# 10XGenomics/thermite

Hardware: AMD Instinct MI355X
Metric: aligned reads/sec (91 bp) (higher is better)
Workload: dtype i32

## Files before the change

thermite_amd/capi.py:

```python
import ctypes as C
import os

import numpy as np

from .refdata import EXON_DT, REF_DT, SPAN_DT, TX_DT

_HERE = os.path.dirname(os.path.abspath(__file__))
SO_PATH = os.environ.get("THM_LIB") or os.path.join(_HERE, "_build", "libthermite_amd.so")

MEM_DT = np.dtype([("ref_idx", "<u8"), ("query_idx", "<u4"), ("len", "<u4")])
ALN_DT = np.dtype(
    [
        ("ystart", "<u8"),
        ("yend", "<u8"),
        ("ylen", "<u8"),
        ("ops_off", "<u8"),
        ("tx_ystart", "<u8"),
        ("tx_yend", "<u8"),
        ("tx_ylen", "<u8"),
        ("tx_ops_off", "<u8"),
        ("score", "<i4"),
        ("ref_id", "<u4"),
        ("xstart", "<u4"),
        ("xend", "<u4"),
# ... 1075 lines not shown
        status = (_copy(v.hit_status, v.n_hits, "<i4") if v.hit_status else np.zeros(int(v.n_hits), "<i4"))
        return _copy(v.alns, v.n_hits, ALN_DT), _copy(v.ops, v.n_op_bytes, np.uint8), status

    def counters(self):
        out = np.zeros(N_COUNTERS, "<u8")
        self._chk(lib().thm_counters_get(self.h, _ptr(out)))
        return out

    def reset_counters(self):
        self._chk(lib().thm_counters_reset(self.h))

    def counters_allreduce(self, comm):
        self._chk(lib().thm_counters_allreduce(self.h, comm.h))

    def counters_device_ptr(self):
        return lib().thm_counters_device_ptr(self.h)

    def timings(self):
        out = np.zeros(N_TIMINGS, "<f4")
        self._chk(lib().thm_timings_get(self.h, _ptr(out)))
        return dict(zip(TIMING_NAMES, out.tolist()))

    def debug_prof(self, reset=True):
        out = np.zeros(16, "<u8")
        self._chk(lib().thm_debug_prof_get(self.h, _ptr(out), int(reset)))
        return out

    def debug_set_pool_caps(self, smem_cap=0, cand_cap=0, ops_cap=0):
        n = C.c_uint32()
        self._chk(lib().thm_debug_set_pool_caps(self.h, smem_cap, cand_cap, ops_cap, C.byref(n)))
        return n.value

    def debug_set_flags(self, tpr=None, rounds=0, seed_infer=None, seed_stats=None, seed_direct=None, finish_exact=None,
                        finish_subst=None):
        word = (0 if tpr is None else (2 if tpr else 1)) | (int(rounds) << 8)
        word |= 0 if seed_infer is None else (16 if seed_infer else 4)
        word |= 0 if seed_stats is None else (8 if seed_stats else 32)
        word |= 0 if seed_direct is None else (128 if seed_direct else 64)
        word |= 0 if finish_exact is None else (0x2000 if finish_exact else 0x1000)
        word |= 0 if finish_subst is None else (0x8000 if finish_subst else 0x4000)
        self._chk(lib().thm_debug_set_flags(self.h, word))

    def debug_seed_stats(self):
        out = np.zeros(2, "<u8")
        self._chk(lib().thm_debug_seed_stats(self.h, _ptr(out)))
        return int(out[0]), int(out[1])

    def debug_smem_finish_stats(self):
        out = np.zeros(4, "<u8")
        self._chk(lib().thm_debug_smem_finish_stats(self.h, _ptr(out)))
        return tuple(int(x) for x in out)

    def debug_seed_direct_stats(self):
        out = np.zeros(4, "<u8")
        self._chk(lib().thm_debug_seed_direct_stats(self.h, _ptr(out)))
        return tuple(int(x) for x in out)

    def debug_fetch_lut(self, like):
        out = np.zeros_like(like)
        self._chk(lib().thm_debug_fetch_lut(self.h, _ptr(out), out.nbytes))
        return out

    def debug_set_band_clip(self, max_bw=None):
        self._chk(lib().thm_debug_set_band_clip(self.h, 0 if max_bw is None else int(max_bw) + 1))

    def debug_tpr_stats(self):
        out = np.zeros(32, "<u8")
        self._chk(lib().thm_debug_tpr_stats(self.h, _ptr(out)))
        return out

    def debug_knobs(self):
        out = np.zeros(16, "<u4")
        self._chk(lib().thm_debug_knobs(self.h, _ptr(out)))
# ... 222 lines not shown
```

thermite_amd/csrc/aligner.hip:

```cpp
#include <hip/hip_runtime.h>

#include <algorithm>
#include <cstdarg>
#include <cstdio>
#include <cstdlib>
#include <cstring>
#include <mutex>
#include <string>
#include <type_traits>
#include <vector>

#include "aligner_internal.h"
#include "lut_direct.h"

namespace thm {
const char* global_error_cstr();
}
using namespace thm;

static int swg_blocks_per_cu() {
  static const int v = [] {
    const char* e = getenv("THM_SWG_BPC");
    const int v = e ? atoi(e) : 4;
    return (v >= 1 && v <= 8) ? v : 4;
// ... 476 lines not shown

int32_t thm_debug_prof_get(thm_aligner* a, uint64_t out[16], int32_t reset) {
  if (!a || !out) return THM_ERR_INVALID_ARG;
  HIPCHK(a, hipSetDevice(a->device));
  unsigned long long* p = a->d_counters + 2 * THM_N_COUNTERS;
  HIPCHK(a, hipMemcpyAsync(out, p, 16 * 8, hipMemcpyDeviceToHost, a->stream));
  if (reset) HIPCHK(a, hipMemsetAsync(p, 0, 16 * 8, a->stream));
  HIPCHK(a, hipStreamSynchronize(a->stream));
  return THM_OK;
}

int32_t thm_debug_set_pool_caps(thm_aligner* a, uint64_t smem_cap, uint64_t cand_cap, uint64_t ops_cap, uint32_t* n_replays) {
  if (!a) return THM_ERR_INVALID_ARG;
  a->dbg_smem_cap = smem_cap;
  a->dbg_cand_cap = cand_cap;
  a->dbg_ops_cap = ops_cap;
  a->seed.smem_cap = a->ext.cand_cap = a->ext.cand_ops_cap = 0;
  if (n_replays) *n_replays = a->n_replays;
  return THM_OK;
}

int32_t thm_debug_set_flags(thm_aligner* a, uint32_t flags) {
  if (!a) return THM_ERR_INVALID_ARG;
  if (flags & 1u) a->tpr.use_tpr = false;
  if (flags & 2u) a->tpr.use_tpr = true;
  const int r = (int)((flags >> 8) & 15u);
  if (r >= 1 && r <= TPR_MAX_ROUNDS) a->tpr.tpr_rounds = r;
  if (flags & 4u) a->dbg_seed_noinfer = true;
  if (flags & 16u) a->dbg_seed_noinfer = false;
  if (flags & 8u) a->dbg_seed_stats = true;
  if (flags & 32u) a->dbg_seed_stats = false;
  if (flags & 64u) a->dbg_seed_nodirect = true;
  if (flags & 128u) a->dbg_seed_nodirect = false;
  if (flags & 0x1000u) a->fin_classes &= ~1u;
  if (flags & 0x2000u) a->fin_classes |= 1u;
  if (flags & 0x4000u) a->fin_classes &= ~2u;
  if (flags & 0x8000u) a->fin_classes |= 2u;
  return THM_OK;
}
int32_t thm_debug_smem_finish_stats(thm_aligner* a, uint64_t stats[4]) {
  if (!a || !stats) return THM_ERR_INVALID_ARG;
  stats[0] = stats[1] = stats[2] = stats[3] = 0;
  if (!a->fin_blocks || !a->ext.finstats.get()) return THM_OK;
  HIPCHK(a, hipSetDevice(a->device));
  HIPCHK(a, hipStreamSynchronize(a->stream));
  std::vector<unsigned long long> rows((size_t)a->fin_blocks * 4);
  HIPCHK(a, hipMemcpy(rows.data(), a->ext.finstats, rows.size() * 8, hipMemcpyDeviceToHost));
  for (size_t b = 0; b < a->fin_blocks; b++)
    for (int k = 0; k < 4; k++) stats[k] += rows[b * 4 + k];
  return THM_OK;
}
int32_t thm_debug_seed_stats(thm_aligner* a, uint64_t stats[2]) {
  if (!a || !stats) return THM_ERR_INVALID_ARG;
  stats[0] = stats[1] = 0;
  if (!a->s_work_counts.p || a->s_work_counts.cap < 128) return THM_OK;
  HIPCHK(a, hipSetDevice(a->device));
  HIPCHK(a, hipStreamSynchronize(a->stream));
  HIPCHK(a, hipMemcpy(stats, a->s_work_counts + 8, 16, hipMemcpyDeviceToHost));
  return THM_OK;
}
int32_t thm_debug_seed_direct_stats(thm_aligner* a, uint64_t stats[4]) {
  if (!a || !stats) return THM_ERR_INVALID_ARG;
  stats[0] = stats[1] = stats[2] = stats[3] = 0;
  if (!a->dix) return THM_OK;
  stats[0] = a->dix->lut_direct ? 1 : 0;
  stats[1] = a->dix->lut_tagged;
// ... 75 lines not shown
```

thermite_amd/csrc/aligner_internal.h:

```cpp
#ifndef THERMITE_ALIGNER_INTERNAL_H
#define THERMITE_ALIGNER_INTERNAL_H
#include <hip/hip_runtime.h>

#include <cstdarg>
#include <cstdio>
#include <string>
#include <type_traits>
#include <vector>

#include "launch.h"
#include "thermite_internal.h"


struct DBuf {
  void* p = nullptr;
  size_t cap = 0;
  DBuf() = default;
  DBuf(const DBuf&) = delete;
  DBuf& operator=(const DBuf&) = delete;
  ~DBuf() { release(); }
  hipError_t ensure(size_t bytes) {
    if (bytes <= cap) return hipSuccess;
    release();
    size_t want = bytes + bytes / 4 + 256;
// ... 333 lines not shown
  Event ev_fork, ev_join;
  thm_align_opts opts;
  thm_align_opts run_opts;
  std::string err;

  DArr<unsigned long long> d_counters;
  DBuf d_ctl;
  static constexpr size_t CTL_WORK_COUNTS = 0, CTL_CURSORS = 128, CTL_FAULT = 192, CTL_QUEUE = 256,
                          CTL_QUEUE_EXT = CTL_QUEUE + thm::QUEUE_BYTES, CTL_BYTES = CTL_QUEUE_EXT + thm::QUEUE_BYTES;
  static_assert(CTL_BYTES % 16 == 0 && thm::QUEUE_BYTES % 16 == 0, "the block is zeroed 16 bytes at a time");
  DView<unsigned int> d_queue;
  DView<unsigned int> d_queue_ext;
  DView<int> d_fault;
  DView<unsigned long long> d_cursors;
  DView<unsigned long long> s_work_counts;
  DBuf b0, b1, b2, b3, b4, b5, b6, b7, b8;
  DArr<uint64_t> stage_scan_tmp;

  ReadsState reads;
  uint64_t n_reads = 0, n_bases = 0;
  uint32_t max_read_len = 0;
  std::vector<std::pair<uint32_t, uint64_t>> len_hist;
  uint64_t n_over = 0;
  bool uploaded = false;
  SeedState seed;
  ExtendState ext;
  uint64_t n_slow_host = 0;
  uint32_t fast_max_len = 0, slow_max_len = 0;
  OutputState out;
  uint64_t dbg_smem_cap = 0, dbg_cand_cap = 0, dbg_ops_cap = 0;
  uint32_t dbg_band_clip = 0;
  bool dbg_seed_noinfer = false, dbg_seed_stats = false;
  bool dbg_seed_nodirect = false;
  uint32_t fin_classes = 3;
  const void* ops_run_ptr = nullptr;
  size_t ops_run_cap = 0;
  uint32_t ops_run_half = 0;
  uint32_t fin_run_classes = 0, fin_blocks = 0;
  uint32_t n_replays = 0;
  bool ran = false, synced = false;
  Event ev[6];
  float timings[THM_N_TIMINGS] = {0};

  std::vector<uint64_t> h_off;
  std::vector<thm_aln> h_alns;
  std::vector<uint8_t> h_ops;
  std::vector<thm_mem> h_mems;
  std::vector<thm_swg_aln> h_swg;
  std::vector<thm_lr_aln> h_lr;
  SeedHitState sh;
  std::vector<thm_aln> h_hit_alns;
  std::vector<int32_t> h_hit_status;
  std::vector<uint8_t> h_hit_ops;
  CigarState cig;
  BamState bam;
  BgzfState bgzf;
  FastqState fq;
  InflateState fz;
  GzipState gz;
};

inline int fail(thm_aligner* a, int code, const char* fmt, ...) {
  char buf[512];
  va_list ap;
  va_start(ap, fmt);
  vsnprintf(buf, sizeof buf, fmt, ap);
// ... 99 lines not shown
```

thermite_amd/csrc/kernels_seed.hip:

```cpp
#include <hip/hip_runtime.h>

#include <algorithm>

#include "launch.h"
#include "lut_direct.h"
#include "swg_device.h"

namespace thm {
namespace dev {

__device__ __forceinline__ int base_code(uint8_t c) {
  return c == 'A' ? 0 : c == 'C' ? 1 : c == 'G' ? 2 : c == 'T' ? 3 : -1;
}
__device__ __forceinline__ uint8_t sanitize_base(uint8_t c) {
  if (c >= 'a' && c <= 'z') c = (uint8_t)(c - 32);
  return (c == 'A' || c == 'C' || c == 'G' || c == 'T' || c == 'N') ? c : (uint8_t)0;
}
__device__ __forceinline__ uint64_t load8_global(const uint8_t* p) {
  uint64_t v;
  __builtin_memcpy(&v, p, 8);
  return v;
}
__device__ __forceinline__ uint64_t load8_lds(const uint8_t* base16, int off) {
  const uint64_t* q = (const uint64_t*)(base16 + (off & ~7));
  const unsigned sh = (unsigned)(off & 7) * 8u;
  const uint64_t w0 = q[0], w1 = q[1];
  return sh ? ((w0 >> sh) | (w1 << (64u - sh))) : w0;
}

template <bool PROBE>
__device__ __forceinline__ int lcp_cmp(const uint8_t* tp, const uint8_t* q, int cap, bool* less) {
  *less = false;
  int o = 0;
  if (PROBE && cap > 0) {
    const uint64_t tw = load8_global(tp), qw = load8_global(q);
    const uint64_t x = tw ^ qw;
    if (x) {
      const int idx = __builtin_ctzll(x) >> 3;
// ... 161 lines not shown

__device__ __forceinline__ void sanitize16(const uint8_t* in, uint8_t* out, uint64_t n, uint64_t n_padded, uint64_t i) {
  if (i >= n_padded) return;
  uint4 v = make_uint4(0, 0, 0, 0);
  if (i < n) v = *(const uint4*)(in + i);
  uint32_t w[4] = {v.x, v.y, v.z, v.w};
#pragma unroll
  for (int j = 0; j < 4; j++) {
    uint32_t r = 0;
#pragma unroll
    for (int b = 0; b < 4; b++) {
      const uint64_t at = i + (uint64_t)(4 * j + b);
      const uint8_t c = (at < n) ? sanitize_base((uint8_t)(w[j] >> (8 * b))) : (uint8_t)0;
      r |= (uint32_t)c << (8 * b);
    }
    w[j] = r;
  }
  *(uint4*)(out + i) = make_uint4(w[0], w[1], w[2], w[3]);
}
__global__ void sanitize_kernel(const uint8_t* in, uint8_t* out, uint64_t n, uint64_t n_padded) {
  sanitize16(in, out, n, n_padded, ((uint64_t)blockIdx.x * blockDim.x + threadIdx.x) * 16);
}
__global__ void sanitize_reset_kernel(const uint8_t* in, uint8_t* out, uint64_t n, uint64_t n_padded, RunResetParams rp) {
  const uint64_t t = (uint64_t)blockIdx.x * blockDim.x + threadIdx.x;
  const uint4 zero = make_uint4(0, 0, 0, 0);
  if (t < rp.status_vec4) rp.status[t] = zero;
  if (t < rp.ctl_vec4) rp.ctl[t] = zero;
  if (t < THM_N_COUNTERS) rp.counters[THM_N_COUNTERS + t] = rp.counters[t];
  if (t == 0) *rp.san_head = zero;
  sanitize16(in, out, n, n_padded, t * 16);
}

constexpr int PROBE_STRIDE = 8;

__device__ __forceinline__ void block_append(bool flag, unsigned long long value, unsigned long long* list,
                                             unsigned long long* count) {
  __shared__ unsigned w_cnt[4];
  __shared__ unsigned long long b_base;
  const unsigned long long m = __ballot(flag);
  const int lane = lane_id(), wv = (int)(threadIdx.x >> 6);
  if (lane == 0) w_cnt[wv] = (unsigned)__popcll(m);
  __syncthreads();
  if (threadIdx.x == 0) {
    const unsigned total = w_cnt[0] + w_cnt[1] + w_cnt[2] + w_cnt[3];
    b_base = total ? atomicAdd(count, (unsigned long long)total) : 0ull;
  }
  __syncthreads();
  unsigned before = 0;
  for (int w = 0; w < wv; w++) before += w_cnt[w];
  if (flag) list[b_base + before + (unsigned long long)__popcll(m & ((1ull << lane) - 1ull))] = value;
  __syncthreads();
}

__device__ __forceinline__ unsigned* seed_stats_lds() {
  __shared__ unsigned s_cnt[4];
  return s_cnt;
}
__device__ __forceinline__ void seed_stats_begin() {
  unsigned* c = seed_stats_lds();
  if (threadIdx.x == 0) c[0] = c[1] = c[2] = c[3] = 0;
  __syncthreads();
}
__device__ __forceinline__ void seed_stats_note(int how) {
  const unsigned long long here = __ballot(1), dec = __ballot(how == MS_DECIDED);
  const unsigned long long dir = __ballot(how == MS_DIRECT), one = __ballot(how == MS_SA_ONE);
  if (lane_id() == (int)__builtin_ctzll(here)) {
    unsigned* c = seed_stats_lds();
    if (dec) atomicAdd(&c[0], (unsigned)__popcll(dec));
    if (here & ~dec) atomicAdd(&c[1], (unsigned)__popcll(here & ~dec));
    if (dir) atomicAdd(&c[2], (unsigned)__popcll(dir));
    if (one) atomicAdd(&c[3], (unsigned)__popcll(one));
  }
}
template <class C>
__device__ __forceinline__ void seed_stats_end(const SeedParamsT<C>& p) {
  unsigned* c = seed_stats_lds();
  __syncthreads();
  if (threadIdx.x == 0) {
    if (c[0]) atomicAdd(&p.work_counts[8], (unsigned long long)c[0]);
    if (c[1]) atomicAdd(&p.work_counts[9], (unsigned long long)c[1]);
    if (c[2]) atomicAdd(&p.work_counts[10], (unsigned long long)c[2]);
    if (c[3]) atomicAdd(&p.work_counts[11], (unsigned long long)c[3]);
  }
}

template <class C>
__device__ __forceinline__ int probe_store(const SeedParamsT<C>& p, const uint8_t* rd, int L, int pos, uint64_t item0, int hint,
                                           bool& decided) {
  const int k = (int)p.min_seed_len;
  int d = 0;
  C lo = 0, hi = 0;
  const int how = ms_search(p.ix, rd, L, pos, k, hint, !(p.flags & SEED_NODIRECT), d, lo, hi);
  decided = how == MS_DECIDED;
  if (p.flags & SEED_STATS) seed_stats_note(how);
  const int e = (d >= k) ? pos + d : 0;
  const uint64_t item = item0 + (uint64_t)pos;
  p.ms_end[item] = (uint16_t)e;
  if (hint == 0 || e > hint) {
    p.ms_lo[item] = lo;
    p.ms_hi[item] = hi;
  }
  return e;
}

template <class C>
__global__ __launch_bounds__(256) void seed_first_kernel(SeedParamsT<C> p) {
  const uint64_t read = (uint64_t)blockIdx.x * 256 + threadIdx.x;
  const int lane = lane_id();
  const bool active = read < p.reads.n_reads;
  const int k = (int)p.min_seed_len;
  if (p.flags & SEED_STATS) seed_stats_begin();
  int d = 0, L = 0, how = MS_FULL;
  C lo = 0, hi = 0;
  bool too_long = false;
  if (active) {
    const uint64_t r0 = p.reads.offsets[read];
    const uint64_t Lfull = p.reads.offsets[read + 1] - r0;
    too_long = Lfull > MAX_READ_LEN;
    L = too_long ? 0 : (int)Lfull;
    if (too_long) p.read_status[read] = THM_ERR_UNSUPPORTED;
    if (k <= L) how = ms_search(p.ix, p.reads.bases + r0, L, 0, k, 0, !(p.flags & SEED_NODIRECT), d, lo, hi);
    if (L > 0) {
      const uint64_t item = ms_row(r0, read);
      p.ms_end[item] = (uint16_t)((d >= k) ? d : 0);
      p.ms_lo[item] = lo;
      p.ms_hi[item] = hi;
    }
// ... 31 lines not shown
      }
      hits = (unsigned long long)(hi - lo);
      p.read_smem_off[read] = slot;
      p.read_smem_cnt[read] = 1u;
      p.read_hits[read] = hits;
    }
    for (int o = 32; o > 0; o >>= 1) hits += __shfl_xor(hits, o);
    if (lane == leader) {
      if (!fits) atomicExch(p.fault, 1);
      atomicAdd(&p.counters[THM_CNT_SMEMS], (unsigned long long)__popcll(m));
      atomicAdd(&p.counters[THM_CNT_HITS], hits);
    }
  }
}

template <class C>
__global__ __launch_bounds__(256) void seed_grid_kernel(SeedParamsT<C> p, const unsigned long long* list,
                                                        const unsigned long long* count, uint32_t G) {
  const uint64_t tid = (uint64_t)blockIdx.x * 256 + threadIdx.x;
  const uint64_t wi = tid / G;
  if (p.flags & SEED_STATS) seed_stats_begin();
  if (wi < *count) {
    const uint64_t read = list[wi];
    const int g = (int)(tid - wi * G);
    const uint64_t r0 = p.reads.offsets[read];
    const int L = (int)(p.reads.offsets[read + 1] - r0);
    const int k = (int)p.min_seed_len;
    const int npos = L - k + 1;
    const int pos = (g + 1 == (int)G) ? npos - 1 : g * PROBE_STRIDE;
    if (!(pos <= 0 || pos >= npos || (g + 1 != (int)G && pos == npos - 1))) {
      const uint64_t item0 = ms_row(r0, read);
      const int hint = (p.flags & SEED_INFER) ? (int)p.ms_end[item0] : 0;
      bool decided;
      (void)probe_store(p, p.reads.bases + r0, L, pos, item0, hint, decided);
    }
  }
  if (p.flags & SEED_STATS) seed_stats_end(p);
}

template <class C>
__global__ __launch_bounds__(256) void seed_grid_cells_kernel(SeedParamsT<C> p, const unsigned long long* list,
                                                              const unsigned long long* count, uint32_t G) {
  __shared__ uint16_t s_end[256];
  const unsigned per = 256u / G;
  const unsigned rl = threadIdx.x / G;
  const int g = (int)(threadIdx.x - rl * G);
  const uint64_t wi = (uint64_t)blockIdx.x * per + rl;
  const bool live = rl < per && wi < *count;
  if (p.flags & SEED_STATS) seed_stats_begin();
  uint64_t read = 0, item0 = 0;
  int npos = 0, e = 0;
  if (live) {
    read = list[wi];
    const uint64_t r0 = p.reads.offsets[read];
    const int L = (int)(p.reads.offsets[read + 1] - r0);
    npos = L - (int)p.min_seed_len + 1;
    item0 = ms_row(r0, read);
    const int pos = (g + 1 == (int)G) ? npos - 1 : g * PROBE_STRIDE;
    const int e0 = p.ms_end[item0];
    if (pos <= 0) {
      e = e0;
    } else if (pos < npos && !(g + 1 != (int)G && pos == npos - 1)) {
      bool decided;
      e = probe_store(p, p.reads.bases + r0, L, pos, item0, (p.flags & SEED_INFER) ? e0 : 0, decided);
    }
  }
  s_end[threadIdx.x] = (uint16_t)e;
  __syncthreads();
  bool todo = false;
  if (live && g + 1 < (int)G) {
    const int a = g * PROBE_STRIDE, b = min(a + PROBE_STRIDE, npos - 1);
    if (b - a > 1) {
      const int ea = e, eb = s_end[rl * G + (unsigned)(b == npos - 1 ? (int)G - 1 : g + 1)];
      if (ea != 0 && ea == eb) {
        for (int q = a + 1; q < b; q++) p.ms_end[item0 + (uint64_t)q] = (uint16_t)ea;
      } else {
        todo = true;
      }
    }
  }
  block_append(todo, (read << 16) | (unsigned long long)g, p.work_cells, &p.work_counts[1]);
  if (p.flags & SEED_STATS) seed_stats_end(p);
}

template <class C>
__global__ __launch_bounds__(256) void seed_cells_kernel(SeedParamsT<C> p, const unsigned long long* list,
                                                         const unsigned long long* count, uint32_t NC) {
  const uint64_t tid = (uint64_t)blockIdx.x * 256 + threadIdx.x;
  const uint64_t wi = tid / NC;
  bool todo = false;
  uint64_t read = 0;
  int c = 0;
  if (wi < *count) {
    read = list[wi];
    c = (int)(tid - wi * NC);
    const uint64_t r0 = p.reads.offsets[read];
    const int L = (int)(p.reads.offsets[read + 1] - r0);
    const int npos = L - (int)p.min_seed_len + 1;
    const int a = c * PROBE_STRIDE, b = min(a + PROBE_STRIDE, npos - 1);
    if (b - a > 1) {
      const uint64_t item0 = ms_row(r0, read);
      const int ea = p.ms_end[item0 + (uint64_t)a], eb = p.ms_end[item0 + (uint64_t)b];
      if (ea != 0 && ea == eb) {
        for (int q = a + 1; q < b; q++) p.ms_end[item0 + (uint64_t)q] = (uint16_t)ea;
      } else {
        todo = true;
      }
    }
  }
  block_append(todo, (read << 16) | (unsigned long long)c, p.work_cells, &p.work_counts[1]);
}

template <class C>
__device__ __forceinline__ bool fill_item(const SeedParamsT<C>& p, uint64_t tid, uint64_t& read, int& pos, uint64_t& r0, int& L) {
  const int j = (int)(tid % PROBE_STRIDE);
  if (j == 0) return false;
  const unsigned long long w = p.work_cells[tid / PROBE_STRIDE];
  read = w >> 16;
  const int c = (int)(w & 0xffffu);
  r0 = p.reads.offsets[read];
  L = (int)(p.reads.offsets[read + 1] - r0);
  const int npos = L - (int)p.min_seed_len + 1;
  pos = c * PROBE_STRIDE + j;
  return pos < min(c * PROBE_STRIDE + PROBE_STRIDE, npos - 1);
}
template <class C>
__device__ __forceinline__ int fill_hint(const SeedParamsT<C>& p, uint64_t item0, int pos) {
  const int steps = ((int)p.min_seed_len + PROBE_STRIDE - 1) / PROBE_STRIDE + 1;
  int a = pos & ~(PROBE_STRIDE - 1);
  for (int s0 = 0; s0 < steps && a >= 0; s0 += 4, a -= 4 * PROBE_STRIDE) {
    int e[4];
#pragma unroll
    for (int u = 0; u < 4; u++) {
      const int at = a - u * PROBE_STRIDE;
      e[u] = (at >= 0 && s0 + u < steps) ? (int)p.ms_end[item0 + (uint64_t)at] : 0;
    }
#pragma unroll
    for (int u = 0; u < 4; u++)
      if (e[u] != 0) return e[u];
  }
  return 0;
}
template <class C>
__device__ __forceinline__ void fill_probe(const SeedParamsT<C>& p, uint64_t read, int pos, uint64_t r0, int L) {
  const uint64_t item0 = ms_row(r0, read);
  const int hint = (p.flags & SEED_INFER) ? fill_hint(p, item0, pos) : 0;
  bool decided;
  (void)probe_store(p, p.reads.bases + r0, L, pos, item0, hint, decided);
}

template <class C>
__global__ __launch_bounds__(256) void seed_fill_kernel(SeedParamsT<C> p) {
  const uint64_t total = p.work_counts[1] * PROBE_STRIDE;
  const uint64_t step = (uint64_t)gridDim.x * 256;
  if (p.flags & SEED_STATS) seed_stats_begin();
  for (uint64_t tid = (uint64_t)blockIdx.x * 256 + threadIdx.x; tid < total; tid += step) {
    uint64_t read, r0;
    int pos, L;
    if (fill_item(p, tid, read, pos, r0, L)) fill_probe(p, read, pos, r0, L);
  }
  if (p.flags & SEED_STATS) seed_stats_end(p);
}

template <class C>
__global__ __launch_bounds__(256) void seed_fill_keys_kernel(SeedParamsT<C> p) {
  const uint64_t total = p.work_counts[1] * PROBE_STRIDE;
  const uint64_t step = (uint64_t)gridDim.x * 256;
  for (uint64_t tid = (uint64_t)blockIdx.x * 256 + threadIdx.x; tid < total; tid += step) {
    uint64_t read, r0;
    int pos, L;
    uint16_t key = 0xFFFF;
    if (fill_item(p, tid, read, pos, r0, L)) {
      const uint64_t w0 = load8_global(p.reads.bases + r0 + pos);
      uint32_t code = 0;
      bool acgt = true;
      for (int t = 0; t < FILL_KEY_BASES; t++) {
        const int c = base_code((uint8_t)((w0 >> (8 * t)) & 0xff));
        acgt = acgt && (c >= 0);
        code = (code << 2) | (uint32_t)(c & 3);
      }
      key = (uint16_t)(acgt ? code : FILL_BUCKETS);
      atomicAdd(&p.fill_hist[key], 1u);
    }
    p.fill_keys[tid] = key;
  }
}
__global__ __launch_bounds__(1024) void seed_fill_scan_kernel(unsigned int* hist) {
  __shared__ unsigned part[1024];
  constexpr unsigned NB = FILL_BUCKETS + 1, PER = (NB + 1023) / 1024;
  const unsigned t = threadIdx.x, b0 = t * PER;
  unsigned sum = 0;
  for (unsigned k = 0; k < PER; k++)
// ... 420 lines not shown
    const uint32_t P = (max_len >= k) ? max_len - k + 1 : 1;
    return (P + dev::PROBE_STRIDE - 1) / dev::PROBE_STRIDE;
  };
  hipError_t e;
  hipLaunchKernelGGL(dev::seed_first_kernel<C>, blocks(n), dim3(256), 0, s, p);
  if ((e = hipGetLastError()) != hipSuccess) return e;
  const uint64_t n_short = n - p.n_long;
  struct Cls {
    uint64_t n;
    uint32_t max_len;
    const unsigned long long* list;
    const unsigned long long* count;
    bool fused;
  } cls[2] = {{n_short, p.max_len_short, p.work_short, p.work_counts + 0, true},
              {p.n_long, p.max_len_long, p.work_long, p.work_counts + 4, false}};
  uint64_t fill_cells = 0;
  for (const Cls& c : cls) {
    if (c.n == 0 || c.max_len < k + 1) continue;
    const uint64_t NC = cells_of(c.max_len), G = NC + 1;
    if (c.fused && G <= 256) {
      const uint64_t per = 256 / G;
      hipLaunchKernelGGL(dev::seed_grid_cells_kernel<C>, dim3((unsigned)((c.n + per - 1) / per)), dim3(256), 0, s, p, c.list, c.count,
                         (uint32_t)G);
      if ((e = hipGetLastError()) != hipSuccess) return e;
    } else {
      hipLaunchKernelGGL(dev::seed_grid_kernel<C>, blocks(c.n * G), dim3(256), 0, s, p, c.list, c.count, (uint32_t)G);
      if ((e = hipGetLastError()) != hipSuccess) return e;
      hipLaunchKernelGGL(dev::seed_cells_kernel<C>, blocks(c.n * NC), dim3(256), 0, s, p, c.list, c.count, (uint32_t)NC);
      if ((e = hipGetLastError()) != hipSuccess) return e;
    }
    fill_cells += c.n * NC;
  }
  if (fill_cells) {
    const dim3 worst = blocks(fill_cells * dev::PROBE_STRIDE);
    const dim3 fixed(std::min<unsigned>(worst.x, 256u * 8u * 4u));
    if (p.fill_mode == 2 && fill_cells * dev::PROBE_STRIDE < (1ull << 32)) {
      hipLaunchKernelGGL(dev::seed_fill_keys_kernel<C>, fixed, dim3(256), 0, s, p);
      hipLaunchKernelGGL(dev::seed_fill_scan_kernel, dim3(1), dim3(1024), 0, s, p.fill_hist);
      hipLaunchKernelGGL(dev::seed_fill_scatter_kernel<C>, fixed, dim3(256), 0, s, p);
      hipLaunchKernelGGL(dev::seed_fill_bucketed_kernel<C>, fixed, dim3(256), 0, s, p);
    } else {
      hipLaunchKernelGGL(dev::seed_fill_kernel<C>, p.fill_mode == 1 ? fixed : worst, dim3(256), 0, s, p);
    }
    if ((e = hipGetLastError()) != hipSuccess) return e;
  }
  auto select_waves = [&](const unsigned long long* list, const unsigned long long* count, unsigned int* queue, uint32_t max_len,
                          int nb) -> hipError_t {
    const uint32_t lcap = sel_lcap(max_len);
    const size_t lds = 4 * (size_t)lcap * (2 * sizeof(C) + 8);
    if (lds <= SEED_SELECT_LDS_LIMIT) {
      hipLaunchKernelGGL((dev::seed_select_kernel<C, false>), dim3(nb), dim3(256), lds, s, p, list, count, queue, lcap);
    } else {
      hipLaunchKernelGGL((dev::seed_select_kernel<C, true>), dim3(nb), dim3(256), 0, s, p, list, count, queue, lcap);
    }
    return hipGetLastError();
  };
  if (n_short) {
    unsigned long long* over_list = p.work_cells;
    unsigned long long* over_count = p.work_counts + 3;
    hipLaunchKernelGGL(dev::seed_select_thread_kernel<C>, dim3((unsigned)((n_short + 255) / 256)), dim3(256),
                       (size_t)256 * (2 * sizeof(C) + 4) * dev::SEL_CAP, s, p, over_list, over_count);
    if ((e = hipGetLastError()) != hipSuccess) return e;
    if ((e = select_waves(over_list, over_count, p.queue, p.max_len_short, std::min(n_blocks, 256))) != hipSuccess) return e;
  }
  if (p.n_long) {
    const int nb = (int)std::min<uint64_t>((uint64_t)n_blocks, (p.n_long + 3) / 4);
    if ((e = select_waves(p.work_long, p.work_counts + 4, p.queue + 1, p.max_len_long, std::max(nb, 1))) != hipSuccess) return e;
  }
  return hipSuccess;
}
hipError_t launch_seed(const SeedParamsT<uint32_t>& p, int n_blocks, hipStream_t s) { return launch_seed_t(p, n_blocks, s); }
hipError_t launch_seed(const SeedParamsT<uint64_t>& p, int n_blocks, hipStream_t s) { return launch_seed_t(p, n_blocks, s); }

template <class C>
static hipError_t launch_plan_pack_t(const PlanParams& pl, const PackParamsT<C>& pk, hipStream_t s) {
// ... 19 lines not shown
```

thermite_amd/csrc/launch.h:

```cpp
#ifndef THERMITE_LAUNCH_H
#define THERMITE_LAUNCH_H

#include <hip/hip_runtime.h>

#include "../../include/thermite_io.h"
#include "extend_plan.h"
#include "thermite_internal.h"

namespace thm {

template <class K, class P>
hipError_t launch_with_lds(K kern, unsigned n_blocks, unsigned threads, size_t lds, hipStream_t s, const P& p) {
  if (lds > 48 * 1024) {
    hipError_t e = hipFuncSetAttribute((const void*)kern, hipFuncAttributeMaxDynamicSharedMemorySize, (int)lds);
    if (e != hipSuccess) return e;
  }
  hipLaunchKernelGGL(kern, dim3(n_blocks), dim3(threads), lds, s, p);
  return hipGetLastError();
}

enum : int { FAULT_OPS_POOL = 1, FAULT_INTERNAL = 2, FAULT_CONTRACT = 4, FAULT_RETRY = 8, FAULT_BAND = 16 };

struct SwgBatchParams {
  const uint8_t* xb;
// ... 57 lines not shown
template <class C>
struct SeedParamsT {
  DeviceIndexT<C> ix;
  ReadBatch reads;
  uint32_t min_seed_len;
  uint32_t max_len_short;
  uint32_t max_len_long;
  uint64_t n_long;
  uint16_t* ms_end;
  C* ms_lo;
  C* ms_hi;
  unsigned long long* work_short;
  unsigned long long* work_long;
  unsigned long long* work_cells;
  unsigned long long* work_counts;
  uint32_t flags;
  SmemT<C>* smems;
  uint64_t smem_cap;
  unsigned long long* cursor;
  uint64_t* read_smem_off;
  uint32_t* read_smem_cnt;
  uint64_t* read_hits;
  int32_t* read_status;
  unsigned long long* counters;
  unsigned int* queue;
  int* fault;
  uint8_t* sel_scratch;
  uint64_t sel_scratch_per_wave;
  uint32_t fill_mode;
  uint16_t* fill_keys;
  uint32_t* fill_perm;
  unsigned int* fill_hist;
};
constexpr uint32_t SEED_INFER = 1u, SEED_STATS = 2u, SEED_NODIRECT = 4u;
constexpr int FILL_KEY_BASES = 7;
constexpr unsigned FILL_BUCKETS = 1u << (2 * FILL_KEY_BASES);
size_t seed_select_lds_bytes(uint32_t max_read_len);
size_t seed_select_scratch_bytes(uint32_t max_read_len);
constexpr size_t SEED_SELECT_LDS_LIMIT = 64 * 1024;
hipError_t launch_seed(const SeedParamsT<uint32_t>& p, int n_blocks, hipStream_t s);
hipError_t launch_seed(const SeedParamsT<uint64_t>& p, int n_blocks, hipStream_t s);
hipError_t launch_sanitize(const uint8_t* in, uint8_t* out, uint64_t n, uint64_t n_padded, hipStream_t s);
hipError_t launch_lut_tag(LutEntryT<uint32_t>* lut, const uint32_t* sa, uint64_t n_entries, uint64_t n, unsigned long long* count, hipStream_t s);
hipError_t launch_lut_tag(LutEntryT<uint64_t>* lut, const uint64_t* sa, uint64_t n_entries, uint64_t n, unsigned long long* count, hipStream_t s);

struct RunResetParams {
  uint4* ctl;
  uint32_t ctl_vec4;
  uint4* status;
  uint64_t status_vec4;
  uint4* san_head;
  unsigned long long* counters;
};
hipError_t launch_sanitize_reset(const uint8_t* in, uint8_t* out, uint64_t n, uint64_t n_padded, const RunResetParams& rp, hipStream_t s);

struct PlanParams {
  const uint64_t* offsets;
  const uint64_t* read_hits;
  uint64_t n_reads;
  uint32_t fast_max_len;
  uint32_t slow_max_len;
  unsigned long long* heavy;
  unsigned long long* slow;
  unsigned long long* team;
  uint32_t team_ok;
  const uint64_t* total_hits;
  uint32_t team_div;
// ... 373 lines not shown
```

thermite_amd/csrc/pipeline.hip:

```cpp
#include <hip/hip_runtime.h>

#include <algorithm>
#include <cstring>

#include "aligner_internal.h"
#include "smem_finish.h"

using namespace thm;

uint32_t seed_fill_mode() {
  static const uint32_t v = [] {
    const char* e = getenv("THM_SEED_FILL");
    const int v = e ? atoi(e) : 0;
    return (uint32_t)(v >= 0 && v <= 2 ? v : 0);
  }();
  return v;
}
unsigned team_div_per_cu() {
  static const unsigned v = [] {
    const char* e = getenv("THM_TEAM_DIV_PER_CU");
    const int v = e ? atoi(e) : 0;
    return v > 0 ? (unsigned)v : TEAM_DIV_PER_CU;
  }();
  return v;
// ... 47 lines not shown
      n_long += lc.second;
    }
  }
  const uint64_t n_short = n - n_long;
  const uint64_t items = ms_row(a->n_bases, n) + 64;
  HIPCHK(a, a->seed.ms_end.ensure(items, 64));
  HIPCHK(a, a->seed.ms_lo.ensure(items * sizeof(C) + 64));
  HIPCHK(a, a->seed.ms_hi.ensure(items * sizeof(C) + 64));
  auto cells_of = [&](uint32_t max_len) -> uint64_t {
    const uint32_t P = (max_len >= min_seed_len) ? max_len - min_seed_len + 1 : 1;
    return (P + 7) / 8;
  };
  const uint64_t cells = n_short * cells_of(max_short) + n_long * cells_of(max_long);
  HIPCHK(a, a->seed.work_reads.ensure(n + 1));
  HIPCHK(a, a->seed.work_long.ensure(n_long + 1));
  HIPCHK(a, a->seed.work_cells.ensure(std::max(cells, n) + 1));
  const int n_blocks = grid_blocks(a, n, 4, lds_blocks_per_cu(std::min(seed_select_lds_bytes(std::max(max_short, 1u)), SEED_SELECT_LDS_LIMIT), 8));
  SeedParamsT<C> sp;
  sp.ix = dev_view<C>(a);
  sp.reads.bases = a->reads.san + 16;
  sp.reads.offsets = a->reads.offsets;
  sp.reads.n_reads = n;
  sp.min_seed_len = min_seed_len;
  sp.max_len_short = max_short;
  sp.max_len_long = max_long;
  sp.n_long = n_long;
  sp.ms_end = a->seed.ms_end;
  sp.ms_lo = a->seed.ms_lo.as<C>();
  sp.ms_hi = a->seed.ms_hi.as<C>();
  sp.work_short = a->seed.work_reads;
  sp.work_long = a->seed.work_long;
  sp.work_cells = a->seed.work_cells;
  sp.work_counts = a->s_work_counts;
  sp.flags = (a->dbg_seed_noinfer ? 0u : SEED_INFER) | (a->dbg_seed_stats ? SEED_STATS : 0u) | (a->dbg_seed_nodirect ? SEED_NODIRECT : 0u);
  sp.smems = a->seed.smems.as<SmemT<C>>();
  sp.smem_cap = a->seed.smem_cap;
  sp.cursor = a->d_cursors;
  sp.read_smem_off = a->seed.off;
  sp.read_smem_cnt = a->seed.cnt;
  sp.read_hits = a->seed.hits;
  sp.read_status = a->reads.status;
  sp.counters = a->d_counters;
  sp.queue = a->d_queue;
  sp.fault = a->d_fault;
  sp.sel_scratch = nullptr;
  sp.sel_scratch_per_wave = 0;
  const uint32_t fill_mode = seed_fill_mode();
  sp.fill_mode = fill_mode;
  sp.fill_keys = nullptr;
  sp.fill_perm = nullptr;
  sp.fill_hist = nullptr;
  if (fill_mode == 2) {
    const uint64_t slots = (std::max(cells, n) + 1) * 8;
    HIPCHK(a, a->seed.fill_keys.ensure(slots));
    HIPCHK(a, a->seed.fill_perm.ensure(slots));
    HIPCHK(a, a->seed.fill_hist.ensure(2 * (FILL_BUCKETS + 1) + 1));
    HIPCHK(a, hipMemsetAsync(a->seed.fill_hist, 0, (2 * (FILL_BUCKETS + 1) + 1) * 4, s));
    sp.fill_keys = a->seed.fill_keys;
    sp.fill_perm = a->seed.fill_perm;
    sp.fill_hist = a->seed.fill_hist;
  }
  if (n_long && seed_select_lds_bytes(max_long) > SEED_SELECT_LDS_LIMIT) {
    const int nb = (int)std::max<uint64_t>(1, std::min<uint64_t>((uint64_t)n_blocks, (n_long + 3) / 4));
    sp.sel_scratch_per_wave = (seed_select_scratch_bytes(max_long) + 255) & ~255ull;
    HIPCHK(a, a->seed.sel_scratch.ensure((size_t)nb * 4 * sp.sel_scratch_per_wave, 256));
    sp.sel_scratch = a->seed.sel_scratch;
  }
// ... 520 lines not shown
```

Before: 96.22 million.

## Use per-probe match-end bounds to skip interior seed fill probes

Each grid probe in the seed stage now records lower and upper bounds on the maximal-match end. Each cell gets a bitmask of the interior positions that still need probing; positions whose end follows from the neighbouring probes' bounds are written directly. The fill kernel compacts the remaining positions per block with a wave scan and LDS before probing, so masked-out positions no longer take a thread. This cuts search probes in the fill pass, at the cost of more complex cell encoding, extra shared memory and block syncs, and a correctness risk if the bounds reasoning is wrong.

```diff
diff --git a/thermite_amd/capi.py b/thermite_amd/capi.py
--- a/thermite_amd/capi.py
+++ b/thermite_amd/capi.py
@@ -1131,13 +1131,14 @@
         return n.value
 
     def debug_set_flags(self, tpr=None, rounds=0, seed_infer=None, seed_stats=None, seed_direct=None, finish_exact=None,
-                        finish_subst=None):
+                        finish_subst=None, seed_bounds=None):
         word = (0 if tpr is None else (2 if tpr else 1)) | (int(rounds) << 8)
         word |= 0 if seed_infer is None else (16 if seed_infer else 4)
         word |= 0 if seed_stats is None else (8 if seed_stats else 32)
         word |= 0 if seed_direct is None else (128 if seed_direct else 64)
         word |= 0 if finish_exact is None else (0x2000 if finish_exact else 0x1000)
         word |= 0 if finish_subst is None else (0x8000 if finish_subst else 0x4000)
+        word |= 0 if seed_bounds is None else (0x20000 if seed_bounds else 0x10000)
         self._chk(lib().thm_debug_set_flags(self.h, word))
 
     def debug_seed_stats(self):
diff --git a/thermite_amd/csrc/aligner.hip b/thermite_amd/csrc/aligner.hip
--- a/thermite_amd/csrc/aligner.hip
+++ b/thermite_amd/csrc/aligner.hip
@@ -532,6 +532,8 @@
   if (flags & 32u) a->dbg_seed_stats = false;
   if (flags & 64u) a->dbg_seed_nodirect = true;
   if (flags & 128u) a->dbg_seed_nodirect = false;
+  if (flags & 0x10000u) a->dbg_seed_nobounds = true;
+  if (flags & 0x20000u) a->dbg_seed_nobounds = false;
   if (flags & 0x1000u) a->fin_classes &= ~1u;
   if (flags & 0x2000u) a->fin_classes |= 1u;
   if (flags & 0x4000u) a->fin_classes &= ~2u;
diff --git a/thermite_amd/csrc/aligner_internal.h b/thermite_amd/csrc/aligner_internal.h
--- a/thermite_amd/csrc/aligner_internal.h
+++ b/thermite_amd/csrc/aligner_internal.h
@@ -389,6 +389,7 @@
   uint32_t dbg_band_clip = 0;
   bool dbg_seed_noinfer = false, dbg_seed_stats = false;
   bool dbg_seed_nodirect = false;
+  bool dbg_seed_nobounds = false;
   uint32_t fin_classes = 3;
   const void* ops_run_ptr = nullptr;
   size_t ops_run_cap = 0;
diff --git a/thermite_amd/csrc/kernels_seed.hip b/thermite_amd/csrc/kernels_seed.hip
--- a/thermite_amd/csrc/kernels_seed.hip
+++ b/thermite_amd/csrc/kernels_seed.hip
@@ -4,6 +4,7 @@
 
 #include "launch.h"
 #include "lut_direct.h"
+#include "seed_bounds.h"
 #include "swg_device.h"
 
 namespace thm {
@@ -231,6 +232,13 @@
 }
 
 constexpr int PROBE_STRIDE = 8;
+static_assert(PROBE_STRIDE == sbd::STRIDE, "seed_bounds.h has the grid stride of the seed stage");
+
+constexpr int CELL_SHIFT = PROBE_STRIDE - 1, READ_SHIFT = CELL_SHIFT + 16;
+constexpr unsigned CELL_ALL = (1u << CELL_SHIFT) - 1u;
+__device__ __forceinline__ unsigned long long cell_item(uint64_t read, int cell, unsigned mask) {
+  return (read << READ_SHIFT) | ((unsigned long long)cell << CELL_SHIFT) | (unsigned long long)mask;
+}
 
 __device__ __forceinline__ void block_append(bool flag, unsigned long long value, unsigned long long* list,
                                              unsigned long long* count) {
@@ -285,13 +293,14 @@
 
 template <class C>
 __device__ __forceinline__ int probe_store(const SeedParamsT<C>& p, const uint8_t* rd, int L, int pos, uint64_t item0, int hint,
-                                           bool& decided) {
+                                           bool& decided, int& la, int& ub) {
   const int k = (int)p.min_seed_len;
   int d = 0;
   C lo = 0, hi = 0;
   const int how = ms_search(p.ix, rd, L, pos, k, hint, !(p.flags & SEED_NODIRECT), d, lo, hi);
   decided = how == MS_DECIDED;
   if (p.flags & SEED_STATS) seed_stats_note(how);
+  sbd::probe_bound(pos, d, !(lo < hi), (int)p.ix.kt, L, la, ub);
   const int e = (d >= k) ? pos + d : 0;
   const uint64_t item = item0 + (uint64_t)pos;
   p.ms_end[item] = (uint16_t)e;
@@ -389,7 +398,8 @@
       const uint64_t item0 = ms_row(r0, read);
       const int hint = (p.flags & SEED_INFER) ? (int)p.ms_end[item0] : 0;
       bool decided;
-      (void)probe_store(p, p.reads.bases + r0, L, pos, item0, hint, decided);
+      int la, ub;
+      (void)probe_store(p, p.reads.bases + r0, L, pos, item0, hint, decided, la, ub);
     }
   }
   if (p.flags & SEED_STATS) seed_stats_end(p);
@@ -399,6 +409,7 @@
 __global__ __launch_bounds__(256) void seed_grid_cells_kernel(SeedParamsT<C> p, const unsigned long long* list,
                                                               const unsigned long long* count, uint32_t G) {
   __shared__ uint16_t s_end[256];
+  __shared__ uint16_t s_ub[256];
   const unsigned per = 256u / G;
   const unsigned rl = threadIdx.x / G;
   const int g = (int)(threadIdx.x - rl * G);
@@ -406,7 +417,7 @@
   const bool live = rl < per && wi < *count;
   if (p.flags & SEED_STATS) seed_stats_begin();
   uint64_t read = 0, item0 = 0;
-  int npos = 0, e = 0;
+  int npos = 0, e = 0, la = 0, ub = 0;
   if (live) {
     read = list[wi];
     const uint64_t r0 = p.reads.offsets[read];
@@ -417,26 +428,36 @@
     const int e0 = p.ms_end[item0];
     if (pos <= 0) {
       e = e0;
+      la = sbd::first_lower_bound(e0);
     } else if (pos < npos && !(g + 1 != (int)G && pos == npos - 1)) {
       bool decided;
-      e = probe_store(p, p.reads.bases + r0, L, pos, item0, (p.flags & SEED_INFER) ? e0 : 0, decided);
+      e = probe_store(p, p.reads.bases + r0, L, pos, item0, (p.flags & SEED_INFER) ? e0 : 0, decided, la, ub);
     }
   }
   s_end[threadIdx.x] = (uint16_t)e;
+  s_ub[threadIdx.x] = (uint16_t)ub;
   __syncthreads();
-  bool todo = false;
+  unsigned mask = 0;
   if (live && g + 1 < (int)G) {
     const int a = g * PROBE_STRIDE, b = min(a + PROBE_STRIDE, npos - 1);
     if (b - a > 1) {
-      const int ea = e, eb = s_end[rl * G + (unsigned)(b == npos - 1 ? (int)G - 1 : g + 1)];
-      if (ea != 0 && ea == eb) {
-        for (int q = a + 1; q < b; q++) p.ms_end[item0 + (uint64_t)q] = (uint16_t)ea;
+      const unsigned sb = rl * G + (unsigned)(b == npos - 1 ? (int)G - 1 : g + 1);
+      if (p.flags & SEED_BOUNDS) {
+        const int k = (int)p.min_seed_len, ubb = s_ub[sb];
+        mask = sbd::cell_mask(a, b, la, ubb, k);
+        for (int q = a + 1; q < b; q++)
+          if (!((mask >> (q - a)) & 1u)) p.ms_end[item0 + (uint64_t)q] = (uint16_t)sbd::decided_end(q, la, ubb, k);
       } else {
-        todo = true;
-      }
-    }
-  }
-  block_append(todo, (read << 16) | (unsigned long long)g, p.work_cells, &p.work_counts[1]);
+        const int ea = e, eb = s_end[sb];
+        if (ea != 0 && ea == eb) {
+          for (int q = a + 1; q < b; q++) p.ms_end[item0 + (uint64_t)q] = (uint16_t)ea;
+        } else {
+          mask = ((1u << (b - a)) - 1u) & ~1u;
+        }
+      }
+    }
+  }
+  block_append(mask != 0, cell_item(read, g, mask >> 1), p.work_cells, &p.work_counts[1]);
   if (p.flags & SEED_STATS) seed_stats_end(p);
 }
 
@@ -465,7 +486,7 @@
       }
     }
   }
-  block_append(todo, (read << 16) | (unsigned long long)c, p.work_cells, &p.work_counts[1]);
+  block_append(todo, cell_item(read, c, CELL_ALL), p.work_cells, &p.work_counts[1]);
 }
 
 template <class C>
@@ -473,8 +494,9 @@
   const int j = (int)(tid % PROBE_STRIDE);
   if (j == 0) return false;
   const unsigned long long w = p.work_cells[tid / PROBE_STRIDE];
-  read = w >> 16;
-  const int c = (int)(w & 0xffffu);
+  if (!((w >> (j - 1)) & 1ull)) return false;
+  read = w >> READ_SHIFT;
+  const int c = (int)((w >> CELL_SHIFT) & 0xffffu);
   r0 = p.reads.offsets[read];
   L = (int)(p.reads.offsets[read + 1] - r0);
   const int npos = L - (int)p.min_seed_len + 1;
@@ -503,18 +525,49 @@
   const uint64_t item0 = ms_row(r0, read);
   const int hint = (p.flags & SEED_INFER) ? fill_hint(p, item0, pos) : 0;
   bool decided;
-  (void)probe_store(p, p.reads.bases + r0, L, pos, item0, hint, decided);
+  int la, ub;
+  (void)probe_store(p, p.reads.bases + r0, L, pos, item0, hint, decided, la, ub);
 }
 
 template <class C>
 __global__ __launch_bounds__(256) void seed_fill_kernel(SeedParamsT<C> p) {
-  const uint64_t total = p.work_counts[1] * PROBE_STRIDE;
+  __shared__ unsigned long long s_item[256];
+  __shared__ uint16_t s_probe[256 * (PROBE_STRIDE - 1)];
+  __shared__ unsigned s_wsum[4];
+  const uint64_t n_cells = p.work_counts[1];
   const uint64_t step = (uint64_t)gridDim.x * 256;
+  const int lane = lane_id(), wv = (int)(threadIdx.x >> 6);
   if (p.flags & SEED_STATS) seed_stats_begin();
-  for (uint64_t tid = (uint64_t)blockIdx.x * 256 + threadIdx.x; tid < total; tid += step) {
-    uint64_t read, r0;
-    int pos, L;
-    if (fill_item(p, tid, read, pos, r0, L)) fill_probe(p, read, pos, r0, L);
+  for (uint64_t c0 = (uint64_t)blockIdx.x * 256; c0 < n_cells; c0 += step) {
+    const unsigned long long w = (c0 + threadIdx.x < n_cells) ? p.work_cells[c0 + threadIdx.x] : 0ull;
+    s_item[threadIdx.x] = w;
+    const unsigned m = (unsigned)w & CELL_ALL;
+    const int cnt = __popc(m);
+    int inc = cnt;
+    for (int o = 1; o < 64; o <<= 1) {
+      const int v = __shfl_up(inc, o);
+      if (lane >= o) inc += v;
+    }
+    if (lane == 63) s_wsum[wv] = (unsigned)inc;
+    __syncthreads();
+    unsigned at = (unsigned)(inc - cnt), total = 0;
+    for (int x = 0; x < 4; x++) {
+      const unsigned v = s_wsum[x];
+      if (x < wv) at += v;
+      total += v;
+    }
+    for (unsigned mm = m; mm; mm &= mm - 1u) s_probe[at++] = (uint16_t)((threadIdx.x << 3) | (unsigned)(__builtin_ctz(mm) + 1));
+    __syncthreads();
+    for (unsigned t = threadIdx.x; t < total; t += 256) {
+      const unsigned pr = s_probe[t];
+      const unsigned long long wc = s_item[pr >> 3];
+      const uint64_t read = wc >> READ_SHIFT;
+      const uint64_t r0 = p.reads.offsets[read];
+      const int L = (int)(p.reads.offsets[read + 1] - r0);
+      const int pos = (int)((wc >> CELL_SHIFT) & 0xffffu) * PROBE_STRIDE + (int)(pr & 7u);
+      if (pos < L - (int)p.min_seed_len) fill_probe(p, read, pos, r0, L);
+    }
+    __syncthreads();
   }
   if (p.flags & SEED_STATS) seed_stats_end(p);
 }
@@ -1001,15 +1054,15 @@
     fill_cells += c.n * NC;
   }
   if (fill_cells) {
-    const dim3 worst = blocks(fill_cells * dev::PROBE_STRIDE);
-    const dim3 fixed(std::min<unsigned>(worst.x, 256u * 8u * 4u));
+    const dim3 worst = blocks(fill_cells);
+    const dim3 fixed(std::min<unsigned>(blocks(fill_cells * dev::PROBE_STRIDE).x, 256u * 8u * 4u));
     if (p.fill_mode == 2 && fill_cells * dev::PROBE_STRIDE < (1ull << 32)) {
       hipLaunchKernelGGL(dev::seed_fill_keys_kernel<C>, fixed, dim3(256), 0, s, p);
       hipLaunchKernelGGL(dev::seed_fill_scan_kernel, dim3(1), dim3(1024), 0, s, p.fill_hist);
       hipLaunchKernelGGL(dev::seed_fill_scatter_kernel<C>, fixed, dim3(256), 0, s, p);
       hipLaunchKernelGGL(dev::seed_fill_bucketed_kernel<C>, fixed, dim3(256), 0, s, p);
     } else {
-      hipLaunchKernelGGL(dev::seed_fill_kernel<C>, p.fill_mode == 1 ? fixed : worst, dim3(256), 0, s, p);
+      hipLaunchKernelGGL(dev::seed_fill_kernel<C>, p.fill_mode == 1 ? dim3(std::min(fixed.x, worst.x)) : worst, dim3(256), 0, s, p);
     }
     if ((e = hipGetLastError()) != hipSuccess) return e;
   }
diff --git a/thermite_amd/csrc/launch.h b/thermite_amd/csrc/launch.h
--- a/thermite_amd/csrc/launch.h
+++ b/thermite_amd/csrc/launch.h
@@ -113,7 +113,7 @@
   uint32_t* fill_perm;
   unsigned int* fill_hist;
 };
-constexpr uint32_t SEED_INFER = 1u, SEED_STATS = 2u, SEED_NODIRECT = 4u;
+constexpr uint32_t SEED_INFER = 1u, SEED_STATS = 2u, SEED_NODIRECT = 4u, SEED_BOUNDS = 8u;
 constexpr int FILL_KEY_BASES = 7;
 constexpr unsigned FILL_BUCKETS = 1u << (2 * FILL_KEY_BASES);
 size_t seed_select_lds_bytes(uint32_t max_read_len);
diff --git a/thermite_amd/csrc/pipeline.hip b/thermite_amd/csrc/pipeline.hip
--- a/thermite_amd/csrc/pipeline.hip
+++ b/thermite_amd/csrc/pipeline.hip
@@ -103,7 +103,8 @@
   sp.work_long = a->seed.work_long;
   sp.work_cells = a->seed.work_cells;
   sp.work_counts = a->s_work_counts;
-  sp.flags = (a->dbg_seed_noinfer ? 0u : SEED_INFER) | (a->dbg_seed_stats ? SEED_STATS : 0u) | (a->dbg_seed_nodirect ? SEED_NODIRECT : 0u);
+  sp.flags = (a->dbg_seed_noinfer ? 0u : SEED_INFER) | (a->dbg_seed_stats ? SEED_STATS : 0u) | (a->dbg_seed_nodirect ? SEED_NODIRECT : 0u) |
+             (a->dbg_seed_nobounds ? 0u : SEED_BOUNDS);
   sp.smems = a->seed.smems.as<SmemT<C>>();
   sp.smem_cap = a->seed.smem_cap;
   sp.cursor = a->d_cursors;
diff --git a/thermite_amd/csrc/seed_bounds.h b/thermite_amd/csrc/seed_bounds.h
--- /dev/null
+++ b/thermite_amd/csrc/seed_bounds.h
@@ -0,0 +1,36 @@
+#ifndef THERMITE_SEED_BOUNDS_H
+#define THERMITE_SEED_BOUNDS_H
+#include <cstdint>
+
+#if defined(__HIPCC__)
+#define SBD_HD __host__ __device__ inline
+#else
+#define SBD_HD inline
+#endif
+
+namespace thm {
+namespace sbd {
+
+constexpr int STRIDE = 8;
+
+SBD_HD void probe_bound(int pos, int d, bool empty, int kt, int L, int& la, int& ub) {
+  if (empty) {
+    la = pos;
+    ub = pos + kt - 1 < L ? pos + kt - 1 : L;
+  } else {
+    la = ub = pos + d;
+  }
+}
+SBD_HD int first_lower_bound(int stored_end) { return stored_end; }
+
+SBD_HD unsigned cell_mask(int a, int b, int la, int ub, int k) {
+  if (la == ub && (a != 0 || ub - b >= k)) return 0u;
+  int n = ub - k - a;
+  if (n > b - a - 1) n = b - a - 1;
+  return n > 0 ? ((1u << n) - 1u) << 1 : 0u;
+}
+SBD_HD int decided_end(int i, int la, int ub, int k) { return (ub - i < k) ? 0 : la; }
+
+}
+}
+#endif
```

Result: faster. 102.1 million (median of 6 runs) (+6.2%).
